# I-Mihara/BioDemuX.jl

Measured on NVIDIA B200. Metric: reads_per_sec, higher is better.
Workload: dtype u32

## Files before the change

biodemux.jl_b200/csrc/api_internal.h:

```cpp
#pragma once

#include <map>
#include <mutex>
#include <string>
#include <vector>

#include "bdx_internal.h"
#include "demux.h"

using namespace bdx;

int bdx_fail(int code, const std::string &msg);
int bdx_cuda_fail(cudaError_t e, const char *what);
std::string &bdx_error_text();
#define CU(call)                                                  \
    do {                                                          \
        cudaError_t e__ = (call);                                 \
        if (e__ != cudaSuccess) return bdx_cuda_fail(e__, #call); \
    } while (0)

struct HostSet {
    int min_m = 0;
    std::vector<uint8_t> bytes, class_of, bc_cls;
    std::vector<int> off, norm, filt_allowed, allowed0;
    std::vector<uint32_t> peq;
    std::vector<uint32_t> pf_bitmap, pf_keys, pf_vals;
    struct HostSeedLevel {
        std::vector<uint32_t> bstart, entries, ekeys, bitmap;
    };
    HostSeedLevel sd[2], sdd[2];
    struct HostSeedVar {
        std::vector<uint16_t> bstart;
        std::vector<uint32_t> entries;
        std::vector<uint8_t> kdepth;
    };
    HostSeedVar sv[2];
    std::vector<uint16_t> hp_bstart, hp_entries;
    std::vector<uint2> hp_bcw;
};

enum { kStepHammingScan, kStepPrefilter, kStepSeed, kStepSeedVar, kStepSeedDeep, kStepFilter, kStepMarkPending,
       kStepLiteral };
enum { kWlNone, kWlWork, kWlWork2 };
enum { kLitAll, kLitCand, kLitWin, kLitFull, kLitRest };
struct PlanStep {
    uint8_t kind, level, in, out, reads, stage;
};
struct PassPlan {
    bool clear_lit = false;
    int n = 0;
    PlanStep step[8];
};
PassPlan plan_pass(const DevParams &P, int pass);
std::string plan_text(const PassPlan &plan);

struct DeviceTables {
    DevParams P;
    PassPlan plan[2];
    std::vector<void *> allocs;
    int sm_count = 0;
};

struct bdx_config {
    uint32_t debug = 0;
    int n_codes = 0;
    uint8_t code_of[256] = {};
    uint8_t rep_of[16] = {};
    DevParams base{};
    HostSet set[2];
    bdx_stats_layout lay{};
    std::mutex mu;
    std::map<int, DeviceTables *> per_device;
};

int bdx_build_set(const bdx_params &p, const bdx_barcode_set &in, HostSet &hs, DevSet &D, uint32_t debug,
                  const char *name);
std::string bdx_describe_set(const HostSet &hs, const DevSet &D);

struct Slot {
    uint8_t *h_seq = nullptr;
    int32_t *h_off = nullptr;
    bdx_result *h_res = nullptr;
    bdx_pass_detail *h_det = nullptr;
    uint8_t *d_packed = nullptr;
    uint8_t *h_packed = nullptr;
    uint8_t *d_win = nullptr;
    int32_t *d_win_off = nullptr;
    int32_t *h_win_off = nullptr;
    uint8_t *d_seq = nullptr;
    int32_t *d_off = nullptr;
    bdx_result *d_res = nullptr;
    bdx_pass_detail *d_det = nullptr;
    cudaEvent_t ev_h2d = nullptr, ev_kern = nullptr, ev_done = nullptr;
    int32_t n = 0;
    uint64_t tag = 0;
    bool busy = false;
    cudaGraphExec_t graph = nullptr;
    int32_t graph_n = -1;
    bool graph_details = false;
    int graph_launches = 0;
    int uses = 0;
};

enum { kStPrefilter = 0, kStSeed = 1, kStSeedDeep = 2, kStFilter = 3, kStLiteral = 4, kStHamming = 5, kStFinalize = 6,
       kStOther = 7 };
struct ProfEvent {
    int kind;
    cudaEvent_t e0, e1;
};

struct bdx_stream {
    bdx_config *cfg = nullptr;
    DeviceTables *tab = nullptr;
    int device = 0;
    int32_t max_reads = 0;
// ... 32 lines not shown
```

biodemux.jl_b200/csrc/bdx_internal.h:

```cpp
#pragma once

#include <cstdint>
#include <cuda_runtime.h>

#include "../../include/bdx.h"

namespace bdx {

constexpr int kMaxBarcodeLen = 256;
constexpr int kMaxFilterWords = 2;
constexpr int kCandMax = 16;
constexpr int kCandOverflow = 255;
constexpr int kCandWindow = 254;
constexpr int kInf = 1 << 29;
constexpr int kMaxCost = 1 << 20;

constexpr int kBcUnknown = 0;
constexpr int kBcAmbiguous = -1;
constexpr int kBcPending = -2;
constexpr int kBcNotRun = -3;

struct DevRange {
    int start_off, start_from_end, end_off, end_from_end;
};

struct SeedLevel {
    int k;
    int q;
    uint32_t pow;
    int log2;
    int bm_log2;
    int n_entries;
    int max_hits;
    const uint32_t *bstart;
    const uint32_t *entries;
    const uint32_t *ekeys;
    const uint32_t *bitmap;
};

struct HammingPacked {
    int enabled;
    int m;
    int allowed;
    int n_seg;
    int n_bstart;
    int seg_off[8], seg_q[8], seg_base[8];
    const uint16_t *bstart;
    const uint16_t *entries;
    const uint2 *bcw;
};

struct SeedVar {
    int enabled;
    int q;
    int q2;
    int bstart2;
    int n_bstart;
    int n_entries;
    int complete;
    int group_reads;
    int hit_rows;
    int qgram_filter;
    double sigma_min;
    const uint16_t *bstart;
    const uint32_t *entries;
    const uint8_t *kdepth;
};

struct DevSet {
    int n_bc;
    int n_bc_pad;
    int max_m;
    int trim_side;
    int words;
    int n_classes;
    int use_filter;
    int pad1;
    DevRange rs, bs, be;
    const uint8_t *bc_bytes;
    const int *bc_off;
    const int *norm;
    const uint32_t *peq;
    const int *filt_allowed;
    const int *allowed0;
    const uint8_t *class_of;
    int pf_enabled;
    int pf_seed;
    uint32_t pf_pow;
    int pf_log2;
    int pf_bm_log2;
    int pad2;
    const uint32_t *pf_bitmap;
    const uint32_t *pf_keys;
    const uint32_t *pf_vals;
    const uint8_t *bc_cls;
    HammingPacked hp;
    int sd_levels;
    int sd_m;
    SeedLevel sd[2];
    int sdd_n;
    int sdd_k;
    SeedLevel sdd[2];
    int sv_levels;
    int pad3;
    SeedVar sv[2];
};

constexpr int kPfMaxSeed = 12;
constexpr int kPfMinSeed = 6;
constexpr uint32_t kPfBase = 0x9E3779B1u;
constexpr uint32_t kPfMix = 0x85EBCA6Bu;
constexpr uint32_t kPfEmpty = 0xFFFFFFFFu;

__host__ __device__ inline uint32_t pf_slot(uint32_t h, int log2size)
{
    return (h * kPfMix) >> (32 - log2size);
}
constexpr uint32_t kPfMix2 = 0xC2B2AE35u;
__host__ __device__ inline uint32_t pf_bit(uint32_t h, int log2bits)
{
    return (h * kPfMix2) >> (32 - log2bits);
}

struct DevParams {
    double max_error_rate, min_delta;
    int match, mismatch, indel, nindel, has_n;
    int algo, is_dual, want_stats;
    int unit_costs;
    int two;
    int debug;
    DevSet set[2];
};

struct PassOut {
    int bc;
    int dist;
    int start, end;
};

constexpr int kStatsOvfCap = 1 << 20;
struct StatsDev {
    unsigned long long *buf;
    bdx_stats_layout lay;
    bdx_stats_overflow *ovf;
    unsigned int *n_ovf;
    unsigned int ovf_cap;
};
// ... 57 lines not shown
```

biodemux.jl_b200/csrc/seed_var.cu:

```cuda
#include <algorithm>
#include <cmath>
#include <cstdlib>
#include <math_constants.h>
#include <type_traits>

#include "bdx_internal.h"
#include "literal.cuh"

namespace bdx {

constexpr int kSvThreads = 128;
constexpr int kSvChains = 2;
constexpr int kSvCand = 8;
constexpr int kSvDiagBias = 64;
constexpr int kSvMaxCols = 180;
constexpr int kSvBig = 1 << 20;
constexpr int kSvRi = 5;

__device__ __forceinline__ void sv_stage_warp(const uint8_t *__restrict__ seq, long long my_start, int my_len,
                                              uint8_t *warp_slots, int stride, const uint8_t *class_s, int lane)
{
    for (int r0 = 0; r0 < 32; r0 += 4) {
        uint32_t w[4][2];
        int mis[4], len[4], nw[4];
#pragma unroll
        for (int j = 0; j < 4; j++) {
            const long long start = __shfl_sync(0xFFFFFFFFu, my_start, r0 + j);
            len[j] = __shfl_sync(0xFFFFFFFFu, my_len, r0 + j);
            const uintptr_t addr = reinterpret_cast<uintptr_t>(seq + start);
            mis[j] = (int)(addr & 3u);
            nw[j] = len[j] ? (mis[j] + len[j] + 3) >> 2 : 0;
            const uint32_t *base = reinterpret_cast<const uint32_t *>(addr - (uintptr_t)mis[j]);
            w[j][0] = lane < nw[j] ? __ldg(base + lane) : 0u;
            w[j][1] = lane + 32 < nw[j] ? __ldg(base + lane + 32) : 0u;
        }
#pragma unroll
        for (int j = 0; j < 4; j++) {
            uint8_t *dst = warp_slots + (size_t)(r0 + j) * stride;
#pragma unroll
            for (int h = 0; h < 2; h++) {
                const int wi = lane + 32 * h;
                if (wi >= nw[j]) continue;
#pragma unroll
                for (int k = 0; k < 4; k++) {
                    const int idx = 4 * wi + k - mis[j];
                    if (idx >= 0 && idx < len[j]) dst[idx] = class_s[(w[j][h] >> (8 * k)) & 0xFFu];
                }
            }
        }
    }
}


enum { kSvPeq = 0, kSvHits, kSvCandL, kSvRinfo, kSvCandN, kSvCtr, kSvBinfo, kSvClass, kSvPlanes, kSvBplanes, kSvSlot, kSvParts };

__host__ __device__ inline int sv_plane_words(int slot_cols, int qgram_filter) { return qgram_filter ? ((slot_cols + 32) / 32 + 3) | 1 : 0; }

__host__ __device__ inline size_t sv_smem_layout(int W, int plane, int n_pad,
                                                 int slot_stride, int R, int hit_rows, int pl_words, size_t off[kSvParts])
{
    size_t o = 0;
    off[kSvPeq] = o; o += (size_t)W * plane * 4;
    off[kSvHits] = o; o += (size_t)kSvThreads * hit_rows * 4;
    off[kSvCandL] = o; o += (size_t)R * kSvCand * 4;
    off[kSvRinfo] = o; o += (size_t)kSvThreads * kSvRi * 4;
    off[kSvCandN] = o; o += ((size_t)kSvThreads + 4) * 4;
    off[kSvCtr] = o; o += 32;
    off[kSvBinfo] = o; o += (size_t)n_pad * 4;
    off[kSvClass] = o; o += 256;
    off[kSvPlanes] = o; o += (size_t)R * 3 * pl_words * 4;
    o = (o + 7) / 8 * 8;
    off[kSvBplanes] = o; o += pl_words ? (size_t)n_pad * 8 : 0;
    off[kSvSlot] = o; o += (size_t)R * slot_stride + 128;
    return (o + 15) / 16 * 16;
}

template <typename WT, bool LASTROW>
__device__ __forceinline__ int sv_verify(const uint32_t *hits_s, int total, const int *rinfo_s, const uint32_t *binfo_s,
                                          const uint32_t *peq_s, int n_classes, int plane, const uint8_t *slot_s,
                                          int slot_stride, uint32_t *cand_s, int *cand_n_s, int seg, const int *cnt)
{
    constexpr int kMsb = (int)sizeof(WT) * 8 - 1;
    const int n0 = seg ? cnt[0] : 0, n1 = seg ? cnt[1] : 0, n2 = seg ? cnt[2] : 0;
    auto fetch = [&](int i) {
        if (seg) {
            int w = 0;
            if (i >= n0) { i -= n0; w = 1; if (i >= n1) { i -= n1; w = 2; if (i >= n2) { i -= n2; w = 3; } } }
            i += w * seg;
        }
        return hits_s[i];
    };
    int cols = 0;
    for (int i0 = 0; i0 < total; i0 += kSvChains * kSvThreads) {
        int score[kSvChains], best[kSvChains], hr[kSvChains], hk[kSvChains], hb[kSvChains], wl[kSvChains], ts[kSvChains];
        WT pv[kSvChains], mv[kSvChains];
        const uint8_t *col[kSvChains];
        const uint32_t *row[kSvChains];
        int wlen = 0;
#pragma unroll
        for (int u = 0; u < kSvChains; u++) {
            const int i = i0 + u * kSvThreads + (int)threadIdx.x;
            const bool live = i < total;
            const uint32_t rec = live ? fetch(i) : 0u;
            hr[u] = live ? (int)(rec >> 22) : 0;
            hb[u] = (int)((rec >> 8) & 0x3FFFu);
            const int delta = (int)(rec & 0xFFu) - kSvDiagBias;
            const uint32_t bi = binfo_s[hb[u]];
            const int m = (int)(bi & 0xFFu);
            hk[u] = live ? (int)((bi >> 8) & 0xFFu) : -1;
            const int Lr = rinfo_s[hr[u] * kSvRi + 0], min_end_rel = rinfo_s[hr[u] * kSvRi + 1];
            const int c0 = live ? max(1, delta - hk[u] + 1) : 1;
            const int c1 = live ? min(Lr, delta + m + hk[u]) : 0;
            wl[u] = c1 - c0 + 1;
            ts[u] = LASTROW ? max(0, min_end_rel - c0) : 0;
            col[u] = slot_s + (size_t)hr[u] * slot_stride + (c0 - 1);
            row[u] = peq_s + hb[u] * n_classes;
            pv[u] = m > kMsb ? ~(WT)0 : (m <= 0 ? (WT)0 : (~(WT)0 << (kMsb + 1 - m)));
            mv[u] = 0;
            score[u] = m;
            best[u] = kInf;
            wlen = max(wlen, wl[u]);
            cols += max(wl[u], 0);
        }
        wlen = __reduce_max_sync(0xFFFFFFFFu, wlen);
#pragma unroll 2
        for (int t = 0; t < wlen; t++) {
            WT eq[kSvChains];
#pragma unroll
            for (int u = 0; u < kSvChains; u++) {
                const uint32_t cls = col[u][t];
                eq[u] = row[u][cls];
                if (sizeof(WT) == 8) eq[u] |= (WT)row[u][plane + cls] << (kMsb - 31);
            }
#pragma unroll
            for (int u = 0; u < kSvChains; u++) {
                int up_prev = 0;
                if (LASTROW) up_prev = score[u] - (int)(pv[u] >> kMsb) + (int)(mv[u] >> kMsb);
                const WT xv = eq[u] | mv[u];
                const WT xh = ((((eq[u] & pv[u]) + pv[u]) ^ pv[u]) | eq[u]);
                const WT ph = mv[u] | ~(xh | pv[u]);
                const WT mh = pv[u] & xh;
                score[u] += (int)(ph >> kMsb) - (int)(mh >> kMsb);
                const WT phs = ph << 1, mhs = mh << 1;
                pv[u] = mhs | ~(xv | phs);
                mv[u] = phs & xv;
                int hit_score = score[u];
                if (LASTROW) {
                    const int up = score[u] - (int)(pv[u] >> kMsb) + (int)(mv[u] >> kMsb);
                    hit_score = min(up + 1, up_prev + 1 - (int)(eq[u] >> kMsb));
                }
                if ((unsigned)(t - ts[u]) < (unsigned)(wl[u] - ts[u])) best[u] = min(best[u], hit_score);
            }
        }
#pragma unroll
        for (int u = 0; u < kSvChains; u++)
            if (hk[u] >= 0 && best[u] <= hk[u]) {
                const int k = atomicAdd(&cand_n_s[hr[u]], 1);
                if (k < kSvCand) cand_s[hr[u] * kSvCand + k] = ((uint32_t)hb[u] << 8) | (uint32_t)best[u];
            }
    }
    return cols;
}

__device__ __forceinline__ bool sv_qgram_pass(const uint32_t *planes_s, int pl_words, const uint2 *bplanes_s, int hr, int b,
                                              int m, int K, int delta)
{
    const int need = (m - 2) - 3 * K;
    if (need <= 0) return true;
    const int biased = delta - K + 32;
    const uint32_t *pl = planes_s + (size_t)hr * 3 * pl_words + (biased >> 5);
    const int sh = biased & 31;
    const uint32_t a_lo = __funnelshift_r(pl[0], pl[1], sh), a_hi = __funnelshift_r(pl[1], pl[2], sh);
    pl += pl_words;
    const uint32_t p_lo = __funnelshift_r(pl[0], pl[1], sh), p_hi = __funnelshift_r(pl[1], pl[2], sh);
    pl += pl_words;
    const uint32_t q_lo = __funnelshift_r(pl[0], pl[1], sh), q_hi = __funnelshift_r(pl[1], pl[2], sh);
    const uint2 bp = bplanes_s[b];
    const uint32_t rows = m >= 32 ? 0xFFFFFFFFu : (1u << m) - 1u;
    uint32_t cover = 0;
    for (int k = 0; k <= 2 * K; k++) {
        const uint32_t mis = (__funnelshift_r(p_lo, p_hi, k) ^ bp.x) | (__funnelshift_r(q_lo, q_hi, k) ^ bp.y) |
                             __funnelshift_r(a_lo, a_hi, k);
        const uint32_t mt = ~mis & rows;
        cover |= mt & (mt >> 1) & (mt >> 2);
    }
    return __popc(cover) >= need;
}

__device__ __forceinline__ int sv_qgram_compact(uint32_t *hits_s, int total, const uint32_t *planes_s, int pl_words,
                                                const uint2 *bplanes_s, const uint32_t *binfo_s, int *cnt, unsigned &n_diag)
{
    static_assert(kSvThreads == 128, "four segments");
    const int lane = threadIdx.x & 31, warp = threadIdx.x >> 5;
    const int seg = ((total + 3) / 4 + 31) & ~31;
    const int s0 = warp * seg, s1 = min(total, s0 + seg);
    int kept = 0;
    for (int i0 = s0; i0 < s1; i0 += 32) {
        const int i = i0 + lane;
        uint32_t rec = 0;
        bool keep = false;
        if (i < s1) {
            rec = hits_s[i];
            const int b = (int)((rec >> 8) & 0x3FFFu);
            const uint32_t bi = binfo_s[b];
            n_diag += 2u * ((bi >> 8) & 0xFFu) + 1u;
            keep = sv_qgram_pass(planes_s, pl_words, bplanes_s, (int)(rec >> 22), b, (int)(bi & 0xFFu), (int)((bi >> 8) & 0xFFu),
                                 (int)(rec & 0xFFu) - kSvDiagBias);
        }
        const uint32_t km = __ballot_sync(0xFFFFFFFFu, keep);
        if (keep) hits_s[s0 + kept + __popc(km & ((1u << lane) - 1u))] = rec;
        kept += __popc(km);
        __syncwarp();
    }
    if (lane == 0) cnt[warp] = kept;
    return seg;
}

template <int W>
__global__ void __launch_bounds__(kSvThreads, 7)
k_seed_var(const __grid_constant__ DevParams P, const int pass, const int level, const uint8_t *__restrict__ seq,
           const int *__restrict__ off, const int n_reads, PassOut *__restrict__ out,
           const PassOut *__restrict__ prev_pass, const int *__restrict__ wl_in, const int *__restrict__ n_in,
           int *__restrict__ wl_out, int *__restrict__ n_out, unsigned long long *__restrict__ counters,
           const int slot_stride, const int slot_cols)
{
    extern __shared__ __align__(16) uint8_t smem_raw[];
    const DevSet &S = P.set[pass];
    const SeedVar &V = S.sv[level];
    const int R = V.group_reads;
    const int n_pad = S.n_bc_pad;
    const int n_classes = S.n_classes;
    const int plane = n_classes * n_pad;
    size_t lo[kSvParts];
    const int pl_words = sv_plane_words(slot_cols, W == 1 && V.qgram_filter);
    sv_smem_layout(W, plane, n_pad, slot_stride, R, V.hit_rows, pl_words, lo);
    uint32_t *peq_s = reinterpret_cast<uint32_t *>(smem_raw + lo[kSvPeq]);
    uint32_t *hits_s = reinterpret_cast<uint32_t *>(smem_raw + lo[kSvHits]);
    uint32_t *cand_s = reinterpret_cast<uint32_t *>(smem_raw + lo[kSvCandL]);
    int *rinfo_s = reinterpret_cast<int *>(smem_raw + lo[kSvRinfo]);
    int *cand_n_s = reinterpret_cast<int *>(smem_raw + lo[kSvCandN]);
    int *ctr_s = reinterpret_cast<int *>(smem_raw + lo[kSvCtr]);
    const uint32_t *entries_s = V.entries;
    const uint16_t *bstart_s = V.bstart;
    uint32_t *binfo_s = reinterpret_cast<uint32_t *>(smem_raw + lo[kSvBinfo]);
    uint8_t *class_s = smem_raw + lo[kSvClass];
    uint8_t *slot_s = smem_raw + lo[kSvSlot];
    uint32_t *planes_s = reinterpret_cast<uint32_t *>(smem_raw + lo[kSvPlanes]);
    uint2 *bplanes_s = reinterpret_cast<uint2 *>(smem_raw + lo[kSvBplanes]);

    for (int k = threadIdx.x; k < W * plane; k += blockDim.x) {
        const int w = k / plane, rem = k - w * plane, c = rem / n_pad, b = rem - c * n_pad;
        peq_s[w * plane + b * n_classes + c] = S.peq[k];
    }
    for (int k = threadIdx.x; k < n_pad; k += blockDim.x) {
        uint32_t v = 0;
        if (k < S.n_bc)
            v = (uint32_t)(S.bc_off[k + 1] - S.bc_off[k]) | ((uint32_t)V.kdepth[k] << 8) |
                ((uint32_t)min(max(S.allowed0[k], 0), 255) << 16);
        binfo_s[k] = v;
    }
    for (int k = threadIdx.x; k < 256; k += blockDim.x) class_s[k] = S.class_of[k];
    if (pl_words)
        for (int k = threadIdx.x; k < n_pad; k += blockDim.x) {
            const int m = k < S.n_bc ? S.bc_off[k + 1] - S.bc_off[k] : 0;
            uint32_t e[5] = {0u, 0u, 0u, 0u, 0u};
            for (int c = 1; c < n_classes && c < 5; c++) e[c] = S.peq[c * n_pad + k];
            const int sh = 32 - m;
            bplanes_s[k] = m >= 1 && m <= 32 ? make_uint2((e[2] | e[4]) >> sh, (e[3] | e[4]) >> sh) : make_uint2(0u, 0u);
        }
    for (int k = threadIdx.x; k < 128; k += blockDim.x) slot_s[(size_t)R * slot_stride + k] = 0;
    if (threadIdx.x == 0) ctr_s[5] = 0;
    __syncthreads();

    using WT = typename std::conditional<W == 1, uint32_t, unsigned long long>::type;
    const int lane = threadIdx.x & 31;
    const int warp = threadIdx.x >> 5;
    const int n_items = wl_in ? *n_in : n_reads;
    const int n_groups = (n_items + R - 1) / R;
    const bool with_delta = P.min_delta != 0.0;
    const int hit_cap = kSvThreads * V.hit_rows;
    const bool in_scan_filter = pl_words && V.qgram_filter == 1;
    const bool dp_fits = V.hit_rows >= S.max_m + 2;
    unsigned int n_done = 0;
    unsigned long long n_cols = 0;
    unsigned long long n_scan = 0;
    unsigned n_diag = 0;

    for (int grp = blockIdx.x; grp < n_groups; grp += gridDim.x) {
        const int item = grp * R + threadIdx.x;
        const bool have = (int)threadIdx.x < R && item < n_items;
        const int read = have ? (wl_in ? wl_in[item] : item) : 0;
        const int base = have ? off[read] : 0;
        const int n = have ? off[read + 1] - base : 0;

        bool punt = !have;
        bool skip = false;
        Geometry g{};
        if (have && pass == 1 && prev_pass[read].bc <= 0) {
            out[read] = PassOut{kBcNotRun, 0, -1, -1};
            skip = true;
            punt = true;
        }
        if (have && !skip) {
            g = pass_geometry(S, n);
            if (!g.valid) {
                out[read] = PassOut{kBcUnknown, 0, -1, -1};
                skip = true;
                punt = true;
            } else if (g.end_j - g.start_j + 1 > slot_cols) {
                punt = true;
            }
        }
        const int sbase = punt ? 0 : g.start_j - 1;
        const int L = punt ? 0 : g.end_j - g.start_j + 1;
        rinfo_s[threadIdx.x * kSvRi + 0] = L;
        rinfo_s[threadIdx.x * kSvRi + 1] = punt ? 1 : max(g.min_end_pos - sbase, -kSvBig);
        rinfo_s[threadIdx.x * kSvRi + 2] = punt ? 0 : min(g.max_start_pos - sbase, kSvBig);
        rinfo_s[threadIdx.x * kSvRi + 3] = 0;
        rinfo_s[threadIdx.x * kSvRi + 4] = n - sbase;
        cand_n_s[threadIdx.x] = 0;
        if (threadIdx.x == 0) ctr_s[0] = 0;
        if (L > 0) atomicMax(&ctr_s[5], L);
        if (warp * 32 < R)
            sv_stage_warp(seq, (long long)base + sbase, L, slot_s + (size_t)warp * 32 * slot_stride, slot_stride, class_s, lane);
        const int last_row_rule = __syncthreads_or(!punt && g.min_end_pos > g.start_j);
        if (pl_words) {
            for (int r = warp; r < R; r += kSvThreads / 32) {
                const int Lr = rinfo_s[r * kSvRi + 0];
                uint32_t *pl = planes_s + (size_t)r * 3 * pl_words;
                for (int w = 0; w < pl_words; w++) {
                    const int c = (w - 1) * 32 + lane;
                    uint32_t a = 0xFFFFFFFFu, b0 = 0u, b1 = 0u;
                    if (w >= 1 && (w - 1) * 32 < Lr) {
                        const uint32_t cls = c < Lr ? slot_s[(size_t)r * slot_stride + c] : 0u;
                        a = __ballot_sync(0xFFFFFFFFu, cls == 0u);
                        b0 = __ballot_sync(0xFFFFFFFFu, cls != 0u && ((cls - 1u) & 1u));
                        b1 = __ballot_sync(0xFFFFFFFFu, cls != 0u && ((cls - 1u) & 2u));
                    }
                    if (lane == 0) {
                        pl[w] = a;
                        pl[pl_words + w] = b0;
                        pl[2 * pl_words + w] = b1;
                    }
                }
            }
            __syncthreads();
        }

        {
            const int q0 = V.q, q1 = V.q2;
            const uint16_t *bst0 = bstart_s, *bst1 = bstart_s + V.bstart2;
            const int n_pos = max(ctr_s[5] - q0 + 1, 0);
            const uint32_t pos_recip = 0xFFFFFFFFu / (uint32_t)max(n_pos, 1) + 1u;
            const int n_pairs = R * n_pos;
            if (threadIdx.x == 0) n_scan += (unsigned)n_pairs;
            for (int base = warp * 64; base < n_pairs; base += (kSvThreads / 32) * 64) {
                uint32_t ea = 0, eb = 0, c4 = 0;
                int lane_total = 0;
#pragma unroll
                for (int u = 0; u < 2; u++) {
                    const int i = base + 2 * lane + u;
                    uint32_t e00 = 0, c00 = 0, e01 = 0, c01 = 0;
                    if (i < n_pairs) {
                        const int r = min((int)__umulhi((uint32_t)i, pos_recip), R - 1), p = i - r * n_pos;
                        const int Lr = rinfo_s[r * kSvRi + 0];
                        if (p + q0 <= Lr) {
                            const uint8_t *c = slot_s + (size_t)r * slot_stride + p;
                            uint32_t code = 0;
                            bool ok = true;
                            for (int k = 0; k < q0; k++) {
                                const uint32_t cl = c[k];
                                ok = ok && cl != 0;
                                code |= ((cl - 1u) & 3u) << (2 * k);
                            }
                            if (ok) {
                                e00 = bst0[code];
                                c00 = bst0[code + 1] - e00;
                                if (q1 && p + q1 <= Lr && c[q0] != 0) {
                                    const uint32_t code1 = code | ((((uint32_t)c[q0] - 1u) & 3u) << (2 * q0));
                                    e01 = bst1[code1];
                                    c01 = bst1[code1 + 1] - e01;
                                }
                            }
                        }
                    }
                    if (u == 0) ea = e00 | (e01 << 16);
                    else eb = e00 | (e01 << 16);
                    c4 |= (c00 | (c01 << 8)) << (16 * u);
                    lane_total += (int)(c00 + c01);
                }
                int incl = lane_total;
#pragma unroll
                for (int o = 1; o < 32; o <<= 1) {
                    const int t = __shfl_up_sync(0xFFFFFFFFu, incl, o);
                    if (lane >= o) incl += t;
                }
                const int total_e = __shfl_sync(0xFFFFFFFFu, incl, 31);
                const int my_excl = incl - lane_total;
                for (int j0 = 0; j0 < total_e; j0 += 32) {
                    const int j = j0 + lane;
                    int ow = 0;
#pragma unroll
                    for (int step = 16; step >= 1; step >>= 1) {
                        const int probe = __shfl_sync(0xFFFFFFFFu, incl, ow + step - 1);
                        if (probe <= j) ow += step;
                    }
                    ow = min(ow, 31);
                    const int o_excl = __shfl_sync(0xFFFFFFFFu, my_excl, ow);
                    const uint32_t oc4 = __shfl_sync(0xFFFFFFFFu, c4, ow);
                    const uint32_t oea = __shfl_sync(0xFFFFFFFFu, ea, ow), oeb = __shfl_sync(0xFFFFFFFFu, eb, ow);
                    bool hit = false;
                    uint32_t rec = 0;
                    int hr = 0;
                    if (j < total_e) {
                        int jj = j - o_excl, which = 0;
                        const int n0 = (int)(oc4 & 0xFFu), n1 = (int)((oc4 >> 8) & 0xFFu), n2 = (int)((oc4 >> 16) & 0xFFu);
                        if (jj >= n0) { jj -= n0; which = 1; if (jj >= n1) { jj -= n1; which = 2; if (jj >= n2) { jj -= n2; which = 3; } } }
                        const uint32_t esel = which < 2 ? oea : oeb;
                        const int e0 = (int)((which & 1) ? (esel >> 16) : (esel & 0xFFFFu));
                        const int oi = base + 2 * ow + (which >> 1);
                        hr = min((int)__umulhi((uint32_t)oi, pos_recip), R - 1);
                        const int op = oi - hr * n_pos;
                        const uint32_t ent = entries_s[e0 + jj];
                        const int b = (int)(ent >> 8), o = (int)(ent & 0xFFu);
                        const uint32_t bi = binfo_s[b];
                        const int m = (int)(bi & 0xFFu), K = (int)((bi >> 8) & 0xFFu), a0 = (int)(bi >> 16);
                        const int oL = rinfo_s[hr * kSvRi + 0], min_end_rel = rinfo_s[hr * kSvRi + 1], max_start_rel = rinfo_s[hr * kSvRi + 2];
                        const int delta = op - o;
                        const int dlo = max(0, min_end_rel - m) - K;
                        const int dhi = min(max_start_rel + a0, oL - m + K);
                        hit = delta >= dlo && delta <= dhi;
                        if (hit && in_scan_filter) {
                            n_diag += 2u * (unsigned)K + 1u;
                            hit = sv_qgram_pass(planes_s, pl_words, bplanes_s, hr, b, m, K, delta);
                        }
                        rec = ((uint32_t)hr << 22) | ((uint32_t)b << 8) | (uint32_t)(delta + kSvDiagBias);
                    }
                    const uint32_t hm = __ballot_sync(0xFFFFFFFFu, hit);
                    if (hm) {
                        int hbase = 0;
                        if (lane == 0) hbase = atomicAdd(&ctr_s[0], __popc(hm));
                        hbase = __shfl_sync(0xFFFFFFFFu, hbase, 0);
                        if (hit) {
                            const int idx = hbase + __popc(hm & ((1u << lane) - 1u));
                            if (idx < hit_cap) hits_s[idx] = rec;
                            else rinfo_s[hr * kSvRi + 3] = 1;
                        }
                    }
                }
            }
        }
        __syncthreads();

        {
            int total = min(ctr_s[0], hit_cap), seg = 0;
            if (pl_words && !in_scan_filter) {
                seg = sv_qgram_compact(hits_s, total, planes_s, pl_words, bplanes_s, binfo_s, ctr_s + 1, n_diag);
                __syncthreads();
                total = ctr_s[1] + ctr_s[2] + ctr_s[3] + ctr_s[4];
            }
            if (last_row_rule)
                n_cols += sv_verify<WT, true>(hits_s, total, rinfo_s, binfo_s, peq_s, n_classes, plane, slot_s, slot_stride, cand_s, cand_n_s, seg, ctr_s + 1);
            else
                n_cols += sv_verify<WT, false>(hits_s, total, rinfo_s, binfo_s, peq_s, n_classes, plane, slot_s, slot_stride, cand_s, cand_n_s, seg, ctr_s + 1);
        }
        __syncthreads();

        const bool usable = !punt && rinfo_s[threadIdx.x * kSvRi + 3] == 0 && cand_n_s[threadIdx.x] <= kSvCand;
        int my_nc = 0;
        uint32_t cl[kSvCand];
        if (usable) {
            const int nc = cand_n_s[threadIdx.x];
#pragma unroll
            for (int k = 0; k < kSvCand; k++) cl[k] = k < nc ? cand_s[threadIdx.x * kSvCand + k] : 0xFFFFFFFFu;
#pragma unroll
            for (int a = 1; a < kSvCand; a++)
#pragma unroll
                for (int bq = a; bq > 0; bq--)
                    if (cl[bq] < cl[bq - 1]) {
                        const uint32_t t = cl[bq];
                        cl[bq] = cl[bq - 1];
                        cl[bq - 1] = t;
                    }
            uint32_t last = 0xFFFFFFFFu;
#pragma unroll
            for (int k = 0; k < kSvCand; k++)
                if (k < nc && (cl[k] >> 8) != last) {
                    last = cl[k] >> 8;
                    cand_s[threadIdx.x * kSvCand + my_nc++] = cl[k];
                }
        }
        const bool start_bound = !punt && g.max_start_pos < n;
        if (__syncthreads_or(start_bound && my_nc > 0)) {
            const Costs c{P.match, P.mismatch, P.indel, P.nindel, P.has_n};
            const WsCol DP{reinterpret_cast<int *>(hits_s) + threadIdx.x, kSvThreads};
            auto check = [&](int r, int k) {
                const uint32_t rec = cand_s[r * kSvCand + k];
                const int b = (int)(rec >> 8), d = (int)(rec & 0xFFu);
                if (!dp_fits) {
                    rinfo_s[r * kSvRi + 3] = 2;
                    return;
                }
                const int qo = S.bc_off[b], m = S.bc_off[b + 1] - qo;
                const int Lr = rinfo_s[r * kSvRi + 0], min_end_rel = rinfo_s[r * kSvRi + 1], max_start_rel = rinfo_s[r * kSvRi + 2];
                const int n_rel = rinfo_s[r * kSvRi + 4];
                const uint8_t *r1 = slot_s + (size_t)r * slot_stride - 1;
                int s_, e_;
                const int dl = sg_literal<false>(DP, DP, S.bc_cls + qo - 1, r1, m, n_rel, d, c, 0, 1, Lr, max_start_rel,
                                                 min_end_rel, s_, e_);
                if (dl != d) rinfo_s[r * kSvRi + 3] = 2;
            };
            if (R > 64) {
                if (start_bound)
                    for (int k = 0; k < my_nc; k++) check(threadIdx.x, k);
            } else {
                const int cnt = start_bound ? my_nc : 0;
                int incl = cnt;
#pragma unroll
                for (int o = 1; o < 32; o <<= 1) {
                    const int t = __shfl_up_sync(0xFFFFFFFFu, incl, o);
                    if (lane >= o) incl += t;
                }
                static_assert(kSvThreads == 128, "four warp totals in ctr_s[1..4]");
                if (lane == 31) ctr_s[1 + warp] = incl;
                __syncthreads();
                int warp_off = 0;
                for (int w = 0; w < warp; w++) warp_off += ctr_s[1 + w];
                int *coff_s = cand_n_s;
                const int total_c = ctr_s[1] + ctr_s[2] + ctr_s[3] + ctr_s[4];
                coff_s[threadIdx.x] = warp_off + incl - cnt;
                __syncthreads();
                for (int j = threadIdx.x; j < total_c; j += kSvThreads) {
                    int lo_r = 0, hi_r = kSvThreads - 1;
                    while (lo_r < hi_r) {
                        const int mid = (lo_r + hi_r + 1) >> 1;
                        if (coff_s[mid] <= j) lo_r = mid;
                        else hi_r = mid - 1;
                    }
                    check(lo_r, j - coff_s[lo_r]);
                }
                __syncthreads();
                cand_n_s[threadIdx.x] = my_nc;
            }
            __syncthreads();
        }
        bool resolved = false;
        if (usable && rinfo_s[threadIdx.x * kSvRi + 3] == 0) {
            const int nc = my_nc;
            BestState bs;
            best_init(bs, P.max_error_rate);
#pragma unroll 1
            for (int k = 0; k < nc; k++) {
                const uint32_t rec = cand_s[threadIdx.x * kSvCand + k];
                const int b = (int)(rec >> 8), d = (int)(rec & 0xFFu);
                const int norm = S.norm[b];
                const int allowed = allowed_from(bs.thr, norm);
                const double sc = d <= allowed ? __ddiv_rn((double)d, (double)norm) : CUDART_INF;
                best_consider(bs, with_delta, sc, d, b + 1, -1, -1);
            }
            if (V.complete) {
                out[read] = best_finish(bs, with_delta, P.min_delta);
                resolved = true;
            } else if (bs.min_bc != 0 && bs.min_score < V.sigma_min) {
                if (!with_delta) {
                    out[read] = best_finish(bs, false, 0.0);
                    resolved = true;
                } else if (__dsub_rn(bs.sub_min, bs.min_score) < P.min_delta) {
                    out[read] = PassOut{kBcAmbiguous, 0, -1, -1};
                    resolved = true;
                } else if (__dsub_rn(V.sigma_min, bs.min_score) >= P.min_delta) {
                    out[read] = PassOut{bs.min_bc, bs.min_dist, -1, -1};
                    resolved = true;
                }
            }
        }
        const bool todo = have && !resolved && !skip;
        const uint32_t mask = __ballot_sync(0xFFFFFFFFu, todo);
        int base_slot = 0;
        if (lane == 0 && mask) base_slot = atomicAdd(n_out, __popc(mask));
        base_slot = __shfl_sync(0xFFFFFFFFu, base_slot, 0);
        if (todo) wl_out[base_slot + __popc(mask & ((1u << lane) - 1u))] = read;
        n_done += __popc(__ballot_sync(0xFFFFFFFFu, resolved));
        if (threadIdx.x == 0) ctr_s[5] = 0;
        __syncthreads();
    }
    if (lane == 0 && n_done && counters) atomicAdd(counters + 2, (unsigned long long)n_done);
    if (counters) {
#pragma unroll
        for (int o = 16; o >= 1; o >>= 1) n_cols += __shfl_down_sync(0xFFFFFFFFu, n_cols, o);
        if (lane == 0 && n_cols) atomicAdd(counters + 3, n_cols);
        unsigned long long nd = n_diag;
#pragma unroll
        for (int o = 16; o >= 1; o >>= 1) nd += __shfl_down_sync(0xFFFFFFFFu, nd, o);
        if (lane == 0 && nd) atomicAdd(counters + 8, nd);
        if (threadIdx.x == 0 && n_scan) atomicAdd(counters + 7, n_scan);
        if (blockIdx.x == 0 && threadIdx.x == 0) atomicAdd(counters + 4, (unsigned long long)n_items);
    }
}

static int sv_slot_cols(const DevSet &S)
{
    const DevRange &r = S.rs;
    if (r.start_from_end == r.end_from_end) {
        const long long len = (long long)r.end_off - r.start_off + 1;
        if (len >= 1 && len <= kSvMaxCols) return (int)len;
        if (len < 1) return 1;
    }
    return kSvMaxCols;
}

struct SvLaunch {
    int slot_cols, slot_stride;
    size_t smem;
};

static SvLaunch sv_launch_params(const DevSet &S, const SeedVar &V)
{
    SvLaunch L;
    L.slot_cols = sv_slot_cols(S);
    int words = (L.slot_cols + 3) / 4;
    words |= 1;
    L.slot_stride = words * 4;
    size_t off[kSvParts];
    const int plane = S.n_classes * S.n_bc_pad;
    L.smem = sv_smem_layout(S.words, plane, S.n_bc_pad, L.slot_stride, V.group_reads, V.hit_rows,
                            sv_plane_words(L.slot_cols, S.words == 1 && V.qgram_filter), off);
    return L;
}

size_t seed_var_smem(const DevSet &S, const SeedVar &V) { return sv_launch_params(S, V).smem; }

cudaError_t launch_seed_var(const DevParams &P, int pass, int level, const uint8_t *seq, const int *off, int n, const Scratch &sc,
                            const int *wl_in, const int *n_in, int *wl_out, int *n_out, int sm_count,
                            unsigned long long *counters, cudaStream_t st)
{
    const DevSet &S = P.set[pass];
    const SeedVar &V = S.sv[level];
    const SvLaunch L = sv_launch_params(S, V);
    auto kern = S.words == 1 ? k_seed_var<1> : k_seed_var<2>;
    int per_sm = 0;
    cudaError_t e = blocks_per_sm_cached((const void *)kern, kSvThreads, L.smem, &per_sm);
    if (e != cudaSuccess) return e;
    const int groups = (n + V.group_reads - 1) / V.group_reads;
    const int blocks = std::max(1, std::min(groups, sm_count * per_sm));
    e = cudaMemsetAsync(n_out, 0, sizeof(int), st);
    if (e != cudaSuccess) return e;
    kern<<<blocks, kSvThreads, L.smem, st>>>(P, pass, level, seq, off, n, sc.pass[pass], sc.pass[0], wl_in, n_in, wl_out, n_out,
                                             counters, L.slot_stride, L.slot_cols);
    return cudaGetLastError();
}

}
```

biodemux.jl_b200/csrc/tables.cu:

```cuda
#include <algorithm>
#include <cmath>
#include <cstdio>
#include <cstring>
#include <string>

#include "api_internal.h"
#include "literal.cuh"

using namespace bdx;

static int narrow_range(const bdx_range &in, DevRange &out, const char *name)
{
    const int64_t lim = 1ll << 30;
    if (in.start_offset > lim || in.start_offset < -lim || in.end_offset > lim || in.end_offset < -lim)
        return bdx_fail(BDX_ERR_INVALID, std::string(name) + ": range offset out of bounds");
    out.start_off = (int)in.start_offset;
    out.start_from_end = in.start_from_end ? 1 : 0;
    out.end_off = (int)in.end_offset;
    out.end_from_end = in.end_from_end ? 1 : 0;
    return BDX_OK;
}

namespace {

// ... 137 lines not shown
            H.ekeys.push_back(pr.second);
        }
    }
    L.n_entries = (int)H.entries.size();
}

void build_seed_levels(const bdx_params &p, HostSet &hs, DevSet &D, uint32_t debug)
{
    if (D.pf_enabled && p.algorithm == BDX_SEMIGLOBAL && D.words >= 1 && hs.min_m == D.max_m && hs.allowed0[0] >= 1 &&
        D.n_bc < (1 << 14) && !(debug & BDX_DEBUG_NO_SEEDS)) {
        const int m = D.max_m, allowed = hs.allowed0[0];
        const double alpha = std::max(2, D.n_classes - 1);
        auto q_of = [&](int k) { return std::min(12, m / (k + 1)); };
        auto rate_of = [&](int k) { return (double)D.n_bc * (k + 1) / std::pow(alpha, q_of(k)); };
        int K = 0;
        for (int k = 1; k <= std::min(allowed, 7); k++)
            if (q_of(k) >= 6 && rate_of(k) <= 0.12) K = k;
        int K0 = 0;
        if (K >= 2 && rate_of(K) > 0.02 && !(debug & BDX_DEBUG_ONE_SEED_LEVEL))
            for (int k = 1; k < K; k++)
                if (rate_of(k) <= 0.01) K0 = k;
        D.sd_m = m;
        for (int K_l : {K0, K}) {
            if (K_l < 1) continue;
            const int l = D.sd_levels++, seg = m / (K_l + 1);
            SeedLevel &L = D.sd[l];
            L.k = K_l;
            L.max_hits = std::max(12, std::min(28, (int)std::ceil(3.0 * 150.0 * rate_of(K_l)) + 2 * (K_l + 1) + 4));
            std::vector<int> offs;
            for (int i = 0; i <= K_l; i++) offs.push_back(i * seg);
            build_hashed_level(hs, D.n_bc, q_of(K_l), offs, L, hs.sd[l]);
        }
    }
}

void build_seed_deep(HostSet &hs, DevSet &D, uint32_t debug)
{
    if (D.sd_levels > 0 && !(debug & BDX_DEBUG_NO_SEED_DEEP)) {
        const int m = D.max_m, allowed = hs.allowed0[0];
        const double alpha = std::max(2, D.n_classes - 1);
        const double deep_rate = 0.25;
        int KD = 0;
        for (int k = D.sd[D.sd_levels - 1].k + 1; k <= std::min(allowed, 7); k++) {
            const int n_seg = k + 1, base_len = m / n_seg, extra = m % n_seg;
            if (base_len < 4) break;
            double rate = 0.0;
            for (int i = 0; i < n_seg; i++) rate += D.n_bc / std::pow(alpha, std::min(base_len + (i < extra ? 1 : 0), 8));
            if (rate <= deep_rate) KD = k;
        }
        if (KD > 0) {
            const int n_seg = KD + 1, base_len = m / n_seg, extra = m % n_seg;
            const int q_long = std::min(base_len + 1, 8), q_short = std::min(base_len, 8);
            D.sdd_k = KD;
            std::vector<int> offs[2];
            int o = 0;
            for (int i = 0; i < n_seg; i++) {
                const int len = base_len + (i < extra ? 1 : 0);
                offs[(std::min(len, 8) == q_long && q_long != q_short) ? 0 : 1].push_back(o);
                o += len;
            }
            for (int t = 0; t < 2; t++) {
                if (offs[t].empty()) continue;
                const int l = D.sdd_n++;
                D.sdd[l].k = KD;
                build_hashed_level(hs, D.n_bc, t == 0 ? q_long : q_short, offs[t], D.sdd[l], hs.sdd[l]);
            }
        }
    }
}

struct VarSeg { int b, o, q; };

bool append_direct_table(const HostSet &hs, int q, const std::vector<VarSeg> &segs, HostSet::HostSeedVar &H)
{
    std::vector<std::vector<uint32_t>> buckets((size_t)1 << (2 * q));
    for (const VarSeg &s : segs) {
        if (s.q != q) continue;
        uint32_t code = 0;
        for (int k = 0; k < q; k++) code |= ((uint32_t)(hs.bc_cls[hs.off[s.b] + s.o + k] - 1) & 3u) << (2 * k);
        buckets[code].push_back(((uint32_t)s.b << 8) | (uint32_t)s.o);
    }
    for (const std::vector<uint32_t> &bk : buckets) {
        if (bk.size() > 255) return false;
        H.bstart.push_back((uint16_t)H.entries.size());
        H.entries.insert(H.entries.end(), bk.begin(), bk.end());
    }
    H.bstart.push_back((uint16_t)H.entries.size());
    return true;
}

void build_seed_var(const bdx_params &p, HostSet &hs, DevSet &D, uint32_t debug)
{
    if (p.algorithm == BDX_SEMIGLOBAL && D.words >= 1 && !p.has_nindel && D.n_classes - 1 <= 4 && D.n_bc < (1 << 14) &&
        D.max_m <= 64 && p.max_error_rate >= 0.0 && !(debug & BDX_DEBUG_NO_SEEDS)) {
        const Geometry g = pass_geometry(D, 150);
        const int L = std::max(g.end_j - g.start_j + 1, 1), sbase = g.start_j - 1;
        const int min_end_rel = g.min_end_pos - sbase, max_start_rel = g.max_start_pos - sbase;
        struct Est { double chance, steps; size_t n_entries; bool complete; };
        auto n_diag = [&](int m, int a0, int K) {
            const int dlo = std::max(0, min_end_rel - m) - K, dhi = std::min(max_start_rel + a0, L - m + K);
            return std::max(0, dhi - dlo + 1);
        };
        auto estimate = [&](int q) {
            Est e{0.0, 0.0, 0, true};
            for (int b = 0; b < D.n_bc; b++) {
                const int m = hs.off[b + 1] - hs.off[b], a0 = hs.allowed0[b];
                const int K = std::min(m / q - 1, a0);
                const double c = (double)(K + 1) * n_diag(m, a0, K) / std::pow(4.0, q);
                e.chance += c;
                e.steps += c * (m + 2 * K);
                e.n_entries += (size_t)K + 1;
                if (K < a0) e.complete = false;
            }
            return e;
        };
        auto size_groups = [&](SeedVar &V, const std::vector<uint8_t> &kdepth, double chance) {
            int strong = 0;
            for (int b = 0; b < D.n_bc; b++)
                strong += (hs.off[b + 1] - hs.off[b] - 2) - 3 * (int)kdepth[(size_t)b] >= 4;
            V.qgram_filter = D.max_m <= 32 && 2 * strong >= D.n_bc && !(debug & BDX_DEBUG_NO_QGRAM_FILTER);
            if (V.qgram_filter) {
                double adm = 0.0, all = 0.0;
                for (int b = 0; b < D.n_bc; b++) {
                    const int m = hs.off[b + 1] - hs.off[b], K = kdepth[(size_t)b];
                    adm += (double)(K + 1) * n_diag(m, hs.allowed0[b], K);
                    all += (double)(K + 1) * L;
                }
                V.qgram_filter = adm >= 0.5 * all ? 1 : 2;
            }
            const double pass = V.qgram_filter == 1 ? (0.15 * strong + (D.n_bc - strong)) / D.n_bc : 1.0;
            const double per_read = chance * pass + 6.0;
            const int per_read_bytes = (L + 8) + (V.qgram_filter ? 12 * ((L + 32) / 32 + 3) : 0) + 64;
            int R = 128;
            while (R > 32 && R * per_read_bytes > 20 * 1024) R -= 32;
            auto rows_for = [&](int r) { return (int)std::ceil(per_read * r / (0.7 * 128)); };
            while (R > 8 && rows_for(R) > 40) R -= R > 32 ? 32 : 8;
            V.group_reads = R;
            V.hit_rows = std::max(8, std::min(40, rows_for(R)));
            const bool can_bound_start = !(D.bs.end_from_end && D.bs.end_off >= 0);
            if (can_bound_start) V.hit_rows = std::max(V.hit_rows, D.max_m + 2);
        };
        auto add_level = [&](int q, const std::vector<VarSeg> &segs, std::vector<uint8_t> kdepth, double chance) {
            HostSet::HostSeedVar &H = hs.sv[D.sv_levels];
            bool two = false;
            for (const VarSeg &s : segs) two = two || s.q != q;
            for (int t = 0; t < (two ? 2 : 1); t++)
                if (!append_direct_table(hs, q + t, segs, H)) {
                    H = HostSet::HostSeedVar();
                    return;
                }
            SeedVar &V = D.sv[D.sv_levels++];
            V.enabled = 1;
            V.q = q;
            V.q2 = two ? q + 1 : 0;
            V.bstart2 = (1 << (2 * q)) + 1;
            V.n_bstart = (int)H.bstart.size();
            V.n_entries = (int)H.entries.size();
            V.complete = 1;
            V.sigma_min = 1e300;
            for (int b = 0; b < D.n_bc; b++) {
                if (kdepth[(size_t)b] < hs.allowed0[b]) V.complete = 0;
                V.sigma_min = std::min(V.sigma_min, (double)(kdepth[(size_t)b] + 1) / (double)hs.norm[b]);
            }
            size_groups(V, kdepth, chance);
            H.kdepth = std::move(kdepth);
        };
        auto build = [&](int q, double chance) {
            std::vector<VarSeg> segs;
            std::vector<uint8_t> kdepth((size_t)D.n_bc);
            for (int b = 0; b < D.n_bc; b++) {
                const int m = hs.off[b + 1] - hs.off[b], K = std::min(m / q - 1, hs.allowed0[b]);
                kdepth[(size_t)b] = (uint8_t)K;
                const int seg = m / (K + 1);
                for (int i = 0; i <= K; i++) segs.push_back(VarSeg{b, i * seg, q});
            }
            add_level(q, segs, std::move(kdepth), chance);
        };
        auto complete_segments = [&](int q_lo, std::vector<VarSeg> &segs) {
            Est e{0.0, 0.0, 0, true};
            for (int b = 0; b < D.n_bc; b++) {
                const int m = hs.off[b + 1] - hs.off[b], a0 = hs.allowed0[b];
                const int n_seg = a0 + 1, base = m / n_seg, extra = m % n_seg;
                int o = 0;
                for (int i = 0; i < n_seg; i++) {
                    const int len = base + (i < extra ? 1 : 0);
                    const int q = (len > q_lo && q_lo < 8) ? q_lo + 1 : q_lo;
                    segs.push_back(VarSeg{b, o, q});
                    const double c = (double)n_diag(m, a0, a0) / std::pow(4.0, q);
                    e.chance += c;
                    e.steps += c * (m + 2 * a0);
                    o += len;
                }
            }
            e.n_entries = segs.size();
            return e;
        };
        int q1 = 0;
        for (int q = 4; q <= 8 && !q1; q++) {
            if (hs.min_m < q) break;
            const Est e = estimate(q);
            if (e.chance <= 24.0 && e.n_entries <= 65535) {
                build(q, e.chance);
                if (D.sv_levels > 0) q1 = q;
            }
        }
        if (q1 && !D.sv[0].complete && !(debug & BDX_DEBUG_ONE_SEED_LEVEL)) {
            int q_lo = 8;
            for (int b = 0; b < D.n_bc; b++) q_lo = std::min(q_lo, (hs.off[b + 1] - hs.off[b]) / (hs.allowed0[b] + 1));
            if (q_lo >= 3) {
                std::vector<VarSeg> segs;
                const Est e = complete_segments(q_lo, segs);
                const double automaton_steps = (double)D.n_bc * L;
                if (e.n_entries <= 65535 && e.steps < 0.5 * automaton_steps && e.chance <= 200.0)
                    add_level(q_lo, segs, std::vector<uint8_t>(hs.allowed0.begin(), hs.allowed0.begin() + D.n_bc), e.chance);
            }
        }
        if (D.sv_levels > 0 && D.sv[D.sv_levels - 1].complete && D.sd_levels == 2 && D.trim_side == 0 && !p.want_stats) {
            const SeedLevel &L2 = D.sd[1];
            const double rate = (double)D.n_bc * (L2.k + 1) / std::pow((double)std::max(2, D.n_classes - 1), L2.q);
            if (rate > 0.02) {
                D.sd[1] = SeedLevel();
                hs.sd[1] = HostSet::HostSeedLevel();
                D.sd_levels = 1;
            }
        }
    }
}

void build_hamming_packed(const bdx_params &p, HostSet &hs, DevSet &D, uint32_t debug)
{
    if (!(debug & BDX_DEBUG_NO_HAMMING_PACKED) && p.algorithm == BDX_HAMMING && hs.min_m == D.max_m && D.max_m <= 32 && D.n_classes - 1 <= 4 && D.n_bc <= 65535 &&
        hs.allowed0[0] >= 0 && hs.allowed0[0] <= 7 && p.max_error_rate >= 0.0 &&
        std::find(hs.bytes.begin(), hs.bytes.end(), (uint8_t)'N') == hs.bytes.end()) {
        const int m = D.max_m, n_seg = hs.allowed0[0] + 1;
        const int seg_len = m / n_seg, extra = m % n_seg;
        if (seg_len >= 2) {
            HammingPacked &H = D.hp;
            H.m = m;
// ... 137 lines not shown
```

Measured before the change: 908.6 million.

## Pack seed bucket start and count into one word; share q-gram codes across pairs

The seed-var bucket table now stores a 32-bit word per bucket holding the start offset and count, so a single load replaces two dependent 16-bit loads. Each lane now builds codes for two adjacent positions from one pass over q0+1 characters instead of two separate loops, and the position count is rounded to even to keep pairs aligned within a row. The q-gram filter call moves out of the hit-decode branch, and optional phase-clock instrumentation is added behind a compile flag. The table grows, the padded positions add a little wasted scan work, and the 16-bit offset packing assumes entries fit in 64K.

```diff
diff --git a/biodemux.jl_b200/csrc/api_internal.h b/biodemux.jl_b200/csrc/api_internal.h
--- a/biodemux.jl_b200/csrc/api_internal.h
+++ b/biodemux.jl_b200/csrc/api_internal.h
@@ -30,7 +30,7 @@
     };
     HostSeedLevel sd[2], sdd[2];
     struct HostSeedVar {
-        std::vector<uint16_t> bstart;
+        std::vector<uint32_t> bstart;
         std::vector<uint32_t> entries;
         std::vector<uint8_t> kdepth;
     };
diff --git a/biodemux.jl_b200/csrc/bdx_internal.h b/biodemux.jl_b200/csrc/bdx_internal.h
--- a/biodemux.jl_b200/csrc/bdx_internal.h
+++ b/biodemux.jl_b200/csrc/bdx_internal.h
@@ -62,7 +62,7 @@
     int hit_rows;
     int qgram_filter;
     double sigma_min;
-    const uint16_t *bstart;
+    const uint32_t *bstart;
     const uint32_t *entries;
     const uint8_t *kdepth;
 };
diff --git a/biodemux.jl_b200/csrc/seed_var.cu b/biodemux.jl_b200/csrc/seed_var.cu
--- a/biodemux.jl_b200/csrc/seed_var.cu
+++ b/biodemux.jl_b200/csrc/seed_var.cu
@@ -16,6 +16,40 @@
 constexpr int kSvMaxCols = 180;
 constexpr int kSvBig = 1 << 20;
 constexpr int kSvRi = 5;
+
+enum { kSvPhStage = 0, kSvPhPlanes, kSvPhPairs, kSvPhPool, kSvPhFilter, kSvPhAppend, kSvPhVerify, kSvPhDecide,
+       kSvPhWorklist, kSvPhases };
+#ifdef BDX_SV_PHASE_CLOCKS
+constexpr int kSvPhLevels = 4;
+__device__ unsigned long long sv_phase_clk[kSvPhLevels][kSvPhases];
+constexpr int kSvPhBytes = kSvThreads / 32 * kSvPhases * 8;
+#define SV_PH_DECL                                                                           \
+    unsigned long long(*sv_ph_s)[kSvPhases] = nullptr;                                       \
+    long long sv_ph_t = 0
+#define SV_PH_INIT()                                                                         \
+    do {                                                                                     \
+        sv_ph_s = reinterpret_cast<unsigned long long(*)[kSvPhases]>(smem_raw + lo[kSvPhClk]); \
+        if (threadIdx.x < kSvThreads / 32 * kSvPhases) (&sv_ph_s[0][0])[threadIdx.x] = 0;    \
+        sv_ph_t = clock64();                                                                 \
+    } while (0)
+#define SV_PH_MARK(ph)                                                                       \
+    do {                                                                                     \
+        const long long sv_ph_now = clock64();                                               \
+        if (lane == 0) sv_ph_s[warp][ph] += (unsigned long long)(sv_ph_now - sv_ph_t);       \
+        sv_ph_t = sv_ph_now;                                                                 \
+    } while (0)
+#define SV_PH_FLUSH()                                                                        \
+    do {                                                                                     \
+        if (lane == 0 && level < kSvPhLevels)                                                \
+            for (int ph = 0; ph < kSvPhases; ph++) atomicAdd(&sv_phase_clk[level][ph], sv_ph_s[warp][ph]); \
+    } while (0)
+#else
+constexpr int kSvPhBytes = 0;
+#define SV_PH_DECL
+#define SV_PH_INIT() do {} while (0)
+#define SV_PH_MARK(ph) do {} while (0)
+#define SV_PH_FLUSH() do {} while (0)
+#endif
 
 __device__ __forceinline__ void sv_stage_warp(const uint8_t *__restrict__ seq, long long my_start, int my_len,
                                               uint8_t *warp_slots, int stride, const uint8_t *class_s, int lane)
@@ -52,7 +86,7 @@
 }
 
 
-enum { kSvPeq = 0, kSvHits, kSvCandL, kSvRinfo, kSvCandN, kSvCtr, kSvBinfo, kSvClass, kSvPlanes, kSvBplanes, kSvSlot, kSvParts };
+enum { kSvPeq = 0, kSvHits, kSvCandL, kSvRinfo, kSvCandN, kSvCtr, kSvBinfo, kSvClass, kSvPlanes, kSvBplanes, kSvSlot, kSvPhClk, kSvParts };
 
 __host__ __device__ inline int sv_plane_words(int slot_cols, int qgram_filter) { return qgram_filter ? ((slot_cols + 32) / 32 + 3) | 1 : 0; }
 
@@ -72,6 +106,8 @@
     o = (o + 7) / 8 * 8;
     off[kSvBplanes] = o; o += pl_words ? (size_t)n_pad * 8 : 0;
     off[kSvSlot] = o; o += (size_t)R * slot_stride + 128;
+    o = (o + 7) / 8 * 8;
+    off[kSvPhClk] = o; o += kSvPhBytes;
     return (o + 15) / 16 * 16;
 }
 
@@ -225,6 +261,7 @@
            const int slot_stride, const int slot_cols)
 {
     extern __shared__ __align__(16) uint8_t smem_raw[];
+    SV_PH_DECL;
     const DevSet &S = P.set[pass];
     const SeedVar &V = S.sv[level];
     const int R = V.group_reads;
@@ -241,12 +278,13 @@
     int *cand_n_s = reinterpret_cast<int *>(smem_raw + lo[kSvCandN]);
     int *ctr_s = reinterpret_cast<int *>(smem_raw + lo[kSvCtr]);
     const uint32_t *entries_s = V.entries;
-    const uint16_t *bstart_s = V.bstart;
+    const uint32_t *bstart_s = V.bstart;
     uint32_t *binfo_s = reinterpret_cast<uint32_t *>(smem_raw + lo[kSvBinfo]);
     uint8_t *class_s = smem_raw + lo[kSvClass];
     uint8_t *slot_s = smem_raw + lo[kSvSlot];
     uint32_t *planes_s = reinterpret_cast<uint32_t *>(smem_raw + lo[kSvPlanes]);
     uint2 *bplanes_s = reinterpret_cast<uint2 *>(smem_raw + lo[kSvBplanes]);
+    SV_PH_INIT();
 
     for (int k = threadIdx.x; k < W * plane; k += blockDim.x) {
         const int w = k / plane, rem = k - w * plane, c = rem / n_pad, b = rem - c * n_pad;
@@ -324,6 +362,7 @@
         if (warp * 32 < R)
             sv_stage_warp(seq, (long long)base + sbase, L, slot_s + (size_t)warp * 32 * slot_stride, slot_stride, class_s, lane);
         const int last_row_rule = __syncthreads_or(!punt && g.min_end_pos > g.start_j);
+        SV_PH_MARK(kSvPhStage);
         if (pl_words) {
             for (int r = warp; r < R; r += kSvThreads / 32) {
                 const int Lr = rinfo_s[r * kSvRi + 0];
@@ -346,48 +385,57 @@
             }
             __syncthreads();
         }
+        SV_PH_MARK(kSvPhPlanes);
 
         {
             const int q0 = V.q, q1 = V.q2;
-            const uint16_t *bst0 = bstart_s, *bst1 = bstart_s + V.bstart2;
-            const int n_pos = max(ctr_s[5] - q0 + 1, 0);
+            const uint32_t *bst0 = bstart_s, *bst1 = bstart_s + V.bstart2;
+            const int n_pos_l = max(ctr_s[5] - q0 + 1, 0);
+            const int n_pos = (n_pos_l + 1) & ~1;
             const uint32_t pos_recip = 0xFFFFFFFFu / (uint32_t)max(n_pos, 1) + 1u;
             const int n_pairs = R * n_pos;
-            if (threadIdx.x == 0) n_scan += (unsigned)n_pairs;
+            if (threadIdx.x == 0) n_scan += (unsigned)(R * n_pos_l);
             for (int base = warp * 64; base < n_pairs; base += (kSvThreads / 32) * 64) {
                 uint32_t ea = 0, eb = 0, c4 = 0;
                 int lane_total = 0;
-#pragma unroll
-                for (int u = 0; u < 2; u++) {
-                    const int i = base + 2 * lane + u;
-                    uint32_t e00 = 0, c00 = 0, e01 = 0, c01 = 0;
-                    if (i < n_pairs) {
-                        const int r = min((int)__umulhi((uint32_t)i, pos_recip), R - 1), p = i - r * n_pos;
-                        const int Lr = rinfo_s[r * kSvRi + 0];
-                        if (p + q0 <= Lr) {
-                            const uint8_t *c = slot_s + (size_t)r * slot_stride + p;
-                            uint32_t code = 0;
-                            bool ok = true;
-                            for (int k = 0; k < q0; k++) {
-                                const uint32_t cl = c[k];
-                                ok = ok && cl != 0;
-                                code |= ((cl - 1u) & 3u) << (2 * k);
-                            }
-                            if (ok) {
-                                e00 = bst0[code];
-                                c00 = bst0[code + 1] - e00;
-                                if (q1 && p + q1 <= Lr && c[q0] != 0) {
-                                    const uint32_t code1 = code | ((((uint32_t)c[q0] - 1u) & 3u) << (2 * q0));
-                                    e01 = bst1[code1];
-                                    c01 = bst1[code1 + 1] - e01;
-                                }
+                const int i = base + 2 * lane;
+                if (i < n_pairs) {
+                    const int r = min((int)__umulhi((uint32_t)i, pos_recip), R - 1), p = i - r * n_pos;
+                    const int Lr = rinfo_s[r * kSvRi + 0];
+                    const uint8_t *c = slot_s + (size_t)r * slot_stride + p;
+                    uint32_t code[2] = {0u, 0u}, ext[2];
+                    bool ok[2] = {true, true};
+                    for (int k = 0; k <= q0; k++) {
+                        const uint32_t cl = c[k], bits = (cl - 1u) & 3u;
+                        if (k < q0) {
+                            ok[0] = ok[0] && cl != 0;
+                            code[0] |= bits << (2 * k);
+                        }
+                        if (k >= 1) {
+                            ok[1] = ok[1] && cl != 0;
+                            code[1] |= bits << (2 * (k - 1));
+                        }
+                    }
+                    ext[0] = c[q0];
+                    ext[1] = c[q0 + 1];
+#pragma unroll
+                    for (int u = 0; u < 2; u++) {
+                        uint32_t e00 = 0, c00 = 0, e01 = 0, c01 = 0;
+                        if (ok[u] && p + u + q0 <= Lr) {
+                            const uint32_t w0 = bst0[code[u]];
+                            e00 = w0 & 0xFFFFu;
+                            c00 = w0 >> 16;
+                            if (q1 && p + u + q1 <= Lr && ext[u] != 0) {
+                                const uint32_t w1 = bst1[code[u] | (((ext[u] - 1u) & 3u) << (2 * q0))];
+                                e01 = w1 & 0xFFFFu;
+                                c01 = w1 >> 16;
                             }
                         }
-                    }
-                    if (u == 0) ea = e00 | (e01 << 16);
-                    else eb = e00 | (e01 << 16);
-                    c4 |= (c00 | (c01 << 8)) << (16 * u);
-                    lane_total += (int)(c00 + c01);
+                        if (u == 0) ea = e00 | (e01 << 16);
+                        else eb = e00 | (e01 << 16);
+                        c4 |= (c00 | (c01 << 8)) << (16 * u);
+                        lane_total += (int)(c00 + c01);
+                    }
                 }
                 int incl = lane_total;
 #pragma unroll
@@ -397,6 +445,7 @@
                 }
                 const int total_e = __shfl_sync(0xFFFFFFFFu, incl, 31);
                 const int my_excl = incl - lane_total;
+                SV_PH_MARK(kSvPhPairs);
                 for (int j0 = 0; j0 < total_e; j0 += 32) {
                     const int j = j0 + lane;
                     int ow = 0;
@@ -411,7 +460,7 @@
                     const uint32_t oea = __shfl_sync(0xFFFFFFFFu, ea, ow), oeb = __shfl_sync(0xFFFFFFFFu, eb, ow);
                     bool hit = false;
                     uint32_t rec = 0;
-                    int hr = 0;
+                    int hr = 0, b = 0, m = 0, K = 0, delta = 0;
                     if (j < total_e) {
                         int jj = j - o_excl, which = 0;
                         const int n0 = (int)(oc4 & 0xFFu), n1 = (int)((oc4 >> 8) & 0xFFu), n2 = (int)((oc4 >> 16) & 0xFFu);
@@ -422,20 +471,25 @@
                         hr = min((int)__umulhi((uint32_t)oi, pos_recip), R - 1);
                         const int op = oi - hr * n_pos;
                         const uint32_t ent = entries_s[e0 + jj];
-                        const int b = (int)(ent >> 8), o = (int)(ent & 0xFFu);
+                        b = (int)(ent >> 8);
+                        const int o = (int)(ent & 0xFFu);
                         const uint32_t bi = binfo_s[b];
-                        const int m = (int)(bi & 0xFFu), K = (int)((bi >> 8) & 0xFFu), a0 = (int)(bi >> 16);
+                        m = (int)(bi & 0xFFu);
+                        K = (int)((bi >> 8) & 0xFFu);
+                        const int a0 = (int)(bi >> 16);
                         const int oL = rinfo_s[hr * kSvRi + 0], min_end_rel = rinfo_s[hr * kSvRi + 1], max_start_rel = rinfo_s[hr * kSvRi + 2];
-                        const int delta = op - o;
+                        delta = op - o;
                         const int dlo = max(0, min_end_rel - m) - K;
                         const int dhi = min(max_start_rel + a0, oL - m + K);
                         hit = delta >= dlo && delta <= dhi;
-                        if (hit && in_scan_filter) {
-                            n_diag += 2u * (unsigned)K + 1u;
-                            hit = sv_qgram_pass(planes_s, pl_words, bplanes_s, hr, b, m, K, delta);
-                        }
                         rec = ((uint32_t)hr << 22) | ((uint32_t)b << 8) | (uint32_t)(delta + kSvDiagBias);
                     }
+                    SV_PH_MARK(kSvPhPool);
+                    if (hit && in_scan_filter) {
+                        n_diag += 2u * (unsigned)K + 1u;
+                        hit = sv_qgram_pass(planes_s, pl_words, bplanes_s, hr, b, m, K, delta);
+                    }
+                    SV_PH_MARK(kSvPhFilter);
                     const uint32_t hm = __ballot_sync(0xFFFFFFFFu, hit);
                     if (hm) {
                         int hbase = 0;
@@ -447,10 +501,12 @@
                             else rinfo_s[hr * kSvRi + 3] = 1;
                         }
                     }
+                    SV_PH_MARK(kSvPhAppend);
                 }
             }
         }
         __syncthreads();
+        SV_PH_MARK(kSvPhAppend);
 
         {
             int total = min(ctr_s[0], hit_cap), seg = 0;
@@ -465,6 +521,7 @@
                 n_cols += sv_verify<WT, false>(hits_s, total, rinfo_s, binfo_s, peq_s, n_classes, plane, slot_s, slot_stride, cand_s, cand_n_s, seg, ctr_s + 1);
         }
         __syncthreads();
+        SV_PH_MARK(kSvPhVerify);
 
         const bool usable = !punt && rinfo_s[threadIdx.x * kSvRi + 3] == 0 && cand_n_s[threadIdx.x] <= kSvCand;
         int my_nc = 0;
@@ -574,6 +631,7 @@
                 }
             }
         }
+        SV_PH_MARK(kSvPhDecide);
         const bool todo = have && !resolved && !skip;
         const uint32_t mask = __ballot_sync(0xFFFFFFFFu, todo);
         int base_slot = 0;
@@ -583,7 +641,9 @@
         n_done += __popc(__ballot_sync(0xFFFFFFFFu, resolved));
         if (threadIdx.x == 0) ctr_s[5] = 0;
         __syncthreads();
-    }
+        SV_PH_MARK(kSvPhWorklist);
+    }
+    SV_PH_FLUSH();
     if (lane == 0 && n_done && counters) atomicAdd(counters + 2, (unsigned long long)n_done);
     if (counters) {
 #pragma unroll
@@ -651,3 +711,18 @@
 }
 
 }
+
+#ifdef BDX_SV_PHASE_CLOCKS
+extern "C" int bdx_sv_phase_clocks(unsigned long long *out, int n, int reset)
+{
+    constexpr int kAll = bdx::kSvPhLevels * bdx::kSvPhases;
+    if (n < kAll) return -1;
+    if (cudaDeviceSynchronize() != cudaSuccess) return -2;
+    if (cudaMemcpyFromSymbol(out, bdx::sv_phase_clk, sizeof(unsigned long long) * kAll) != cudaSuccess) return -2;
+    if (reset) {
+        static const unsigned long long zero[kAll] = {};
+        if (cudaMemcpyToSymbol(bdx::sv_phase_clk, zero, sizeof zero) != cudaSuccess) return -2;
+    }
+    return kAll;
+}
+#endif
diff --git a/biodemux.jl_b200/csrc/tables.cu b/biodemux.jl_b200/csrc/tables.cu
--- a/biodemux.jl_b200/csrc/tables.cu
+++ b/biodemux.jl_b200/csrc/tables.cu
@@ -243,10 +243,9 @@
     }
     for (const std::vector<uint32_t> &bk : buckets) {
         if (bk.size() > 255) return false;
-        H.bstart.push_back((uint16_t)H.entries.size());
+        H.bstart.push_back((uint32_t)H.entries.size() | ((uint32_t)bk.size() << 16));
         H.entries.insert(H.entries.end(), bk.begin(), bk.end());
     }
-    H.bstart.push_back((uint16_t)H.entries.size());
     return true;
 }
 
@@ -314,7 +313,7 @@
             V.enabled = 1;
             V.q = q;
             V.q2 = two ? q + 1 : 0;
-            V.bstart2 = (1 << (2 * q)) + 1;
+            V.bstart2 = 1 << (2 * q);
             V.n_bstart = (int)H.bstart.size();
             V.n_entries = (int)H.entries.size();
             V.complete = 1;
```

After: 915.3 million, median of 6. Within noise of the previous version (+0.7%).
